# NVIDIA/cuopt

Measured on AMD Instinct MI355X. Metric: pdlp_iterations_per_sec, higher is better.
Workload: dtype f64; 1 GPU; c3: synthetic random sparse LP S(m=1000000,n=1000000,k=10,seed=2), nnz=10000000, longest row 10, CSR fp64/int32, Stable2 preset, tolerances 0 (fixed iteration budget); rows=1000000, cols=1000000, nnz=10000000, parallelism=single GPU

## Files before the change

cuopt_amd/csrc/pdlp_create.hip:

```cpp
#include "pdlp_ctx.hpp"
#include "pdlp_layouts.hpp"
#include "pdlp_setup.hpp"

__global__ void k_fill(int64_t n, double* __restrict__ d, double v);
int sync_panel_values(pdlpdev_ctx* c);
int resident_tier(int m, int n, int64_t nnz);

static thread_local int g_create_sharded = 0;
static thread_local int g_create_no_resident = 0;
static thread_local int g_create_batch_lanes = 0;

static int create_impl(pdlpdev_ctx** out, int device, int32_t m, int32_t n, const int32_t* a_offsets,
                       const int32_t* a_indices, const double* a_values, const int32_t* at_offsets,
                       const int32_t* at_indices, const double* at_values,
                       void (*transpose_ready)(void*), void* user, const double* c, const double* lo,
                       const double* hi, const double* lb, const double* ub, pdlpdev_analysis* an);

extern "C" {

const char* pdlpdev_last_error(void) { return g_err.c_str(); }
void pdlpdev_create_hint(int sharded) { g_create_sharded = sharded; }
void pdlpdev_create_no_resident(int no_resident) { g_create_no_resident = no_resident; }
void pdlpdev_create_batch_lanes(int lanes) { g_create_batch_lanes = lanes; }
static thread_local pdlpdev_ctx* g_create_stream_donor = nullptr;
// ... 446 lines not shown
    lap("wait for the A^T side");
    if ((int64_t)at_offsets[n] != ctx->nnz) return fail(-1, "pdlpdev_create: A and A^T disagree on nnz");
    if (!an) {
      TRY(upload_i32(ctx, &ctx->At.full.off, at_offsets, (size_t)n + 1));
      TRY(upload_i32(ctx, &ctx->At.full.idx, at_indices, nnz, 8));
      TRY(upload_f64(ctx, &ctx->At.full.val, at_values, nnz, 8));
    }
    ctx->At.nlong = (int)lat.size();
    if (ctx->At.nlong) TRY(upload_i32(ctx, &ctx->At.longs, lat.data(), lat.size()));
    const bool hot_t = !hT_off.empty();
    ctx->At.hot = ctx->At.full;
    ctx->At.hot_nnz = (int64_t)T.off[n];
    if (hot_t) {
      TRY(upload_i32(ctx, &ctx->At.hot.off, T.off, (size_t)n + 1));
      TRY(upload_i32(ctx, &ctx->At.hot.idx, T.idx, (size_t)ctx->At.hot_nnz, 8));
      TRY(dev_alloc(ctx, &ctx->At.hot.val, (size_t)ctx->At.hot_nnz + 8));
      TRY(upload_i32(ctx, &ctx->dense.s_perm_at, hT_perm.data(), hT_perm.size()));
    }
    if (DH.on) TRY(dev_alloc(ctx, &ctx->At.dense_add, (size_t)n));
    ctx->At.nb = (int)rbt.size() / 2 - 1;
    TRY(upload_i32(ctx, &ctx->At.rb, rbt.data(), rbt.size()));
    lap("upload A^T");
    T.d_off = ctx->At.hot.off, T.d_idx = ctx->At.hot.idx, T.d_val = ctx->At.hot.val;
    TRY(at_thread ? at_rc : layout_walk(ctx, P, T));
    TRY(upload_side(ctx, P, T));
    if (ctx->At.pan.on && DH.on) TRY(column_segments(ctx, DH, T.ph));
    lap("upload layouts A^T");
    HIP_TRY(hipStreamSynchronize(ctx->stream));
  }
  {
    const char* small_env = getenv("CUOPT_AMD_SMALL");
    const int tier        = resident_tier(m, n, ctx->nnz);
    ctx->eval_reuse_aty   = cuopt_amd::tune_int("eval_reuse_aty", 1) != 0;
    ctx->small_resident   = tier >= 0 && !(small_env && atoi(small_env) == 0) && !ctx->A.dense_add && !ctx->At.dense_add && !g_create_no_resident;
    g_create_no_resident  = 0;
    if (small_env && atoi(small_env) != 0 && tier < 0)
      return fail(-1, "CUOPT_AMD_SMALL=1: the LP does not fit the resident kernel (m, n <= 2048, nnz <= 4096 ...)");
  }
  ctx->slab_cap += slab_rest;
  for (pdlpdev_ctx::MatrixSide* s : {&ctx->A, &ctx->At}) {
    s->pan.v.dense_add = s->jag.v.dense_add = s->pb.v.dense_add = s->dense_add;
    if (s->pan.v.dn_own_seg || s->pan.v.dn_pan_ptr) s->pan.v.dense_add = nullptr;
  }
  TRY(lp_alloc_partials(ctx));
  lap("partial buffers");
  k_fill<<<grid_for(m), kBlock, 0, ctx->stream>>>(m, ctx->dr, 1.0);
  k_fill<<<grid_for(n), kBlock, 0, ctx->stream>>>(n, ctx->dc, 1.0);
  HIP_TRY(hipGetLastError());
  lap("fill D");
  TRY(sync_panel_values(ctx));
  lap("panel values (permute)");
  if (P.mode == LayoutPolicy::kTimed) {
    TRY(pick_layout(ctx, &ctx->A, ctx->tmp_n, ctx->tmp_m));
    lap("layout autotune A");
    TRY(pick_layout(ctx, &ctx->At, ctx->tmp_m, ctx->tmp_n));
    lap("layout autotune");
  }
  if (one_gpu && !ctx->small_resident && ctx->A.layout() == pdlpdev_ctx::MatrixSide::kPanel && !ctx->A.pan.v.seg && cuopt_amd::tune_int("zero_skip", 1) != 0) {
    const size_t words = 2 * (((size_t)n + 127) / 128);
    ctx->zs_mode = cuopt_amd::tune_int("zero_skip", 1) == 2 ? 2 : 1;
    TRY(dev_alloc(ctx, &ctx->zcount, (size_t)grid_for(n)));
    TRY(dev_alloc(ctx, &ctx->xmask, words + 2));
    HIP_TRY(hipMemsetAsync(ctx->xmask, 0, (words + 2) * sizeof(unsigned long long), ctx->stream));
  }
  HIP_TRY(hipStreamSynchronize(ctx->stream));
  scratch_free(ctx);
// ... 34 lines not shown
```

cuopt_amd/csrc/pdlp_ctx.hpp:

```cpp
#pragma once
#include <hip/hip_runtime.h>
#include <hip/hip_ext.h>

#include <tuple>
#include <utility>

#include <dlfcn.h>
#include <unistd.h>
#include <mutex>
#include <math.h>
#include <stdarg.h>
#include <stdio.h>
#include <string.h>

#include <algorithm>
#include <chrono>
#include <map>
#include <memory>
#include <string>
#include <vector>

#include "host_parallel.hpp"
#include "pdlp_kernels.hpp"
#include "pdlp_epilogues.hpp"
// ... 296 lines not shown
    }
    int max_partials() const { return std::max({nb, pb.on ? pb.v.B : 0, pan.on ? pan.v.W : 0, jag.on ? jag.v.nblk + jag.v.nlong : 0, 1}); }
    void info(int32_t out[3]) const
    {
      out[0] = layout();
      switch (layout()) {
        case kPb: out[1] = pb.v.B, out[2] = (int)(100.0 * (pb.pad - 1.0) + 0.5); break;
        case kJag: out[1] = jag.v.nblk, out[2] = (int)(100.0 * jag.saving + 0.5); break;
        case kPanel: out[1] = pan.v.W, out[2] = pan.v.S; break;
        default: out[1] = nb, out[2] = 1;
      }
    }
    bool fuses_dense() const { return pan.on && (pan.v.dn_own_seg != nullptr || pan.v.dn_pan_ptr != nullptr); }
  };
  MatrixSide A, At;
  struct Dense {
    bool on = false;
    int nrows = 0, nseg = 0, ntiles = 0;
    int64_t nent = 0;
    int32_t *row = nullptr, *row_seg = nullptr;
    int32_t *seg_row = nullptr, *seg_c0 = nullptr, *seg_len = nullptr, *seg_ptr = nullptr;
    int32_t *ch_seg = nullptr, *ch_k0 = nullptr, *row_ch = nullptr;
    double* ch_part = nullptr;
    int nchunks = 0;
    int32_t *tile_ptr = nullptr, *tile_seg = nullptr, *tile_id = nullptr;
    int32_t *perm = nullptr, *s_perm_a = nullptr, *s_perm_at = nullptr;
    double* val = nullptr;
    int32_t* tile_slot = nullptr;
  } dense;
  double *c = nullptr, *c_u = nullptr;
  double *dr = nullptr, *dc = nullptr;
  bool scaled = false;
  int eval_reuse_aty = 1;
  int batch_lanes = 0;
  bool small_resident = false;
  rccl::comm_t comm = nullptr;
  softcomm::Comm* soft = nullptr;
  std::string comm_key;
  int rank = 0, world = 1;
  bool rsag = false;
  int slice = 0;
  double* rs_buf = nullptr;
  double* rs_scal = nullptr;
  bool owner = false;
  int ypad = 0;
  double* ygather = nullptr;
  MatrixSide Oc;
  struct Halo {
    bool on = false;
    std::vector<int32_t> recv_off[2], recv_cnt[2], send_off[2], send_cnt[2];
    int64_t bytes = 0, bytes_allgather = 0;
  } halo;
  struct P2P {
    bool on = false;
    char* base = nullptr;
    size_t bytes = 0;
    size_t off_x = 0, off_y = 0, off_s = 0, off_f = 0;
    p2pdev::Peers peers{};
    std::vector<void*> opened;
    unsigned long long* epoch = nullptr;
    int* fault = nullptr;
    p2pdev::Push* push_dev = nullptr;
    p2pdev::Push push_host[p2pdev::kKinds];
  } p2p;
};

struct HalpernBurstStats { int64_t bursts = 0, periods = 0, records = 0, empty = 0; };

struct CtxLp {
  double *lb = nullptr, *ub = nullptr, *lo = nullptr, *hi = nullptr;
  double *lb_u = nullptr, *ub_u = nullptr, *lo_u = nullptr, *hi_u = nullptr;
  double *x[2] = {nullptr, nullptr}, *y[2] = {nullptr, nullptr}, *aty[2] = {nullptr, nullptr};
  double *xbar = nullptr, *sumx = nullptr, *sumy = nullptr, *avgx = nullptr, *avgy = nullptr;
  unsigned long long* xmask = nullptr;
  int* zcount = nullptr;
  int zs_mode = 0;
  double *lrx = nullptr, *lry = nullptr, *rc[2] = {nullptr, nullptr};
  double *tmp_n = nullptr, *tmp_m = nullptr;
  double *ax_u[3] = {nullptr, nullptr, nullptr}, *aty_u[3] = {nullptr, nullptr, nullptr};
  double* rc_scratch = nullptr;
  double *bestx = nullptr, *besty = nullptr, *bestrc = nullptr;
  double *part_g = nullptr;
  double *scal = nullptr;
  double *scal_h = nullptr;
  pdlpdev_ctl *ctl = nullptr, *ctl_h = nullptr;
  pdlpdev_step_params sp = {0.3, 0.6, 0.5, 0.5};
  bool halpern = false;
  double* lraty = nullptr;
  pdlpdev_halpern *hal = nullptr, *hal_h = nullptr;
  bool halpern_rays = false;
  struct pdlpdev_halpern_major_state* hmaj = nullptr;
  pdlpdev_halpern_major_record* hmaj_ring = nullptr;
  HalpernBurstStats burst_stats;
  double* ar_buf = nullptr;
  bool prof_armed = false;
  static constexpr int kProfPairs = 8;
  hipEvent_t prof_ev[2 * kProfPairs] = {};
  int prof_used = 0;
  int rejected_in_a_row = 0;
  bool aty_valid = false, ctl_h_current = false;
  bool batch_ctl_fresh = false;
  int batch_ray_steps = -1, batch_ray_rule = -1;
  int64_t stat_single_rays = 0;
  int spare_attempts = 0;
  int64_t stat_eval_reused = 0, stat_eval_product = 0, stat_loop_syncs = 0, stat_empty_attempts = 0;
  int64_t stat_scaling[2][9] = {};
  int use_graph = 1;
  bool comm_warm = false;
  bool graph_comm_failed = false;
// ... 261 lines not shown
```

cuopt_amd/csrc/pdlp_device.hip:

```cpp
#include "pdlp_ctx.hpp"
#include "pdlp_layouts.hpp"
#include "pdlp_setup.hpp"
#include "halpern_decision.hpp"


__global__ void __launch_bounds__(kBlock) k_fill(int64_t n, double* __restrict__ d, double v)
{
  for (int64_t i = blockIdx.x * (int64_t)kBlock + threadIdx.x; i < n; i += (int64_t)gridDim.x * kBlock)
    d[i] = v;
}
__global__ void __launch_bounds__(kBlock) k_scale_vectors(int n, int m, double* __restrict__ c,
                                                          double* __restrict__ lb,
                                                          double* __restrict__ ub,
                                                          const double* __restrict__ dc,
                                                          double* __restrict__ lo,
                                                          double* __restrict__ hi,
                                                          const double* __restrict__ dr)
{
  const int tot = n > m ? n : m;
  for (int i = blockIdx.x * kBlock + threadIdx.x; i < tot; i += gridDim.x * kBlock) {
    if (i < n) {
      c[i]  = c[i] * dc[i];
      lb[i] = lb[i] / dc[i];
      ub[i] = ub[i] / dc[i];
// ... 52 lines not shown
    } else if (MODE == 1) {
      acc[0] += a[i] * a[i];
    } else if (MODE == 2) {
      const double v = combine_bounds(a[i], b[i]);
      acc[0] += v * v;
    } else {
      const double v = a[i] - b[i];
      acc[0] += v * v;
    }
  }
  if (MODE == 0)
    block_reduce<MaxOp, 1>(acc, red);
  else
    block_reduce<SumOp, 1>(acc, red);
  if (threadIdx.x == 0) part[blockIdx.x] = acc[0];
}
__global__ void __launch_bounds__(kBlock) k_dot(int64_t n, const double* __restrict__ a, const double* __restrict__ b,
                                                double* __restrict__ part)
{
  __shared__ double red[8];
  double acc[1] = {0.0};
  for (int64_t i = blockIdx.x * (int64_t)kBlock + threadIdx.x; i < n; i += (int64_t)gridDim.x * kBlock) acc[0] += a[i] * b[i];
  block_reduce<SumOp, 1>(acc, red);
  if (threadIdx.x == 0) part[blockIdx.x] = acc[0];
}
__global__ void __launch_bounds__(kBlock) k_finalize(const double* __restrict__ part, int nb, int nq,
                                                     unsigned op_mask, double* __restrict__ out)
{
  __shared__ double red[8];
  finalize_rows(part, nb, nq, op_mask, out, red);
}

template <bool ZS>
__device__ __forceinline__ void
primal_body(int n, const pdlpdev_ctl* __restrict__ ctl, double* __restrict__ x0, double* __restrict__ x1,
         const double* __restrict__ aty0, const double* __restrict__ aty1,
         const double* __restrict__ c, const double* __restrict__ lb, const double* __restrict__ ub,
         double* __restrict__ xbar, double* __restrict__ sumx, const p2pdev::Push* __restrict__ push, pdlpdev_ctx::UniformBounds ubd,
         unsigned long long* __restrict__ xmask, int* __restrict__ zcount)
{
  [[maybe_unused]] int nz = 0;
  if (!loop_active(ctl)) return;
  const int cur       = ctl->cur;
  const double tau    = ctl->tau;
  const double weight = ctl->step_size;
  const bool pend     = ctl->pending_avg != 0;
  const double* __restrict__ x   = cur ? x1 : x0;
  double* __restrict__ xn        = cur ? x0 : x1;
  const double* __restrict__ aty = cur ? aty1 : aty0;
  for (int j = blockIdx.x * kBlock + threadIdx.x; j < n; j += gridDim.x * kBlock) {
    const double xj       = x[j];
    const double gradient = c[j] - aty[j];
    double next           = xj - (tau * gradient);
    next                  = dmax(dmin(next, ubd.ub_same ? ubd.ub : ub[j]), ubd.lb_same ? ubd.lb : lb[j]);
    xn[j]                 = next;
    const double xb       = next - xj + next;
    xbar[j]               = xb;
    if constexpr (ZS) {
      const unsigned long long bits = __ballot(xb != 0.0);
      if ((threadIdx.x & 63) == 0) xmask[j >> 6] = bits;
      nz += __popcll(bits);
    }
    if (push)
      for (int q = 0; q < push->world; ++q)
        if (push->wants(q, j)) p2pdev::put(push->slot(q) + j, xb);
    if (pend) sumx[j] = sumx[j] + weight * xj;
  }
  if constexpr (ZS) {
    __shared__ int wave_nz[kBlock / 64];
    if ((threadIdx.x & 63) == 0) wave_nz[threadIdx.x >> 6] = nz;
    __syncthreads();
    if (threadIdx.x == 0) {
      int sum = 0;
#pragma unroll
      for (int w = 0; w < kBlock / 64; ++w) sum += wave_nz[w];
      zcount[blockIdx.x] = sum;
    }
  }
  if (push) p2pdev::count_exchange(push);
}
__global__ void __launch_bounds__(kBlock)
k_primal(int n, const pdlpdev_ctl* __restrict__ ctl, double* __restrict__ x0, double* __restrict__ x1,
         const double* __restrict__ aty0, const double* __restrict__ aty1,
         const double* __restrict__ c, const double* __restrict__ lb, const double* __restrict__ ub,
         double* __restrict__ xbar, double* __restrict__ sumx, const p2pdev::Push* __restrict__ push, pdlpdev_ctx::UniformBounds ubd)
{
  primal_body<false>(n, ctl, x0, x1, aty0, aty1, c, lb, ub, xbar, sumx, push, ubd, nullptr, nullptr);
}
__global__ void __launch_bounds__(kBlock)
k_primal_zs(int n, const pdlpdev_ctl* __restrict__ ctl, double* __restrict__ x0, double* __restrict__ x1,
            const double* __restrict__ aty0, const double* __restrict__ aty1,
            const double* __restrict__ c, const double* __restrict__ lb, const double* __restrict__ ub,
            double* __restrict__ xbar, double* __restrict__ sumx, pdlpdev_ctx::UniformBounds ubd,
            unsigned long long* __restrict__ xmask, int* __restrict__ zcount)
{
  primal_body<true>(n, ctl, x0, x1, aty0, aty1, c, lb, ub, xbar, sumx, nullptr, ubd, xmask, zcount);
}



__global__ void __launch_bounds__(kBlock)
k_step_stats(int n, int nbg, const pdlpdev_ctl* __restrict__ ctl, const double* __restrict__ reduced,
             const double* __restrict__ x0, const double* __restrict__ x1, double* __restrict__ aty0,
             double* __restrict__ aty1, double* __restrict__ part)
{
  __shared__ double red[12];
  if (!loop_active(ctl)) return;
  const int cur = ctl->cur;
  const double* __restrict__ x   = cur ? x1 : x0;
  const double* __restrict__ xn  = cur ? x0 : x1;
  const double* __restrict__ aty = cur ? aty1 : aty0;
  double* __restrict__ atyn      = cur ? aty0 : aty1;
  double acc[2] = {0.0, 0.0};
  for (int j = blockIdx.x * kBlock + threadIdx.x; j < n; j += gridDim.x * kBlock) {
    const double v  = reduced[j];
    atyn[j]         = v;
    const double dx = xn[j] - x[j];
    const double t  = v - aty[j];
    acc[0] += t * dx;
    acc[1] += dx * dx;
  }
  block_reduce<SumOp, 2>(acc, red);
  if (threadIdx.x == 0) {
    part[blockIdx.x]       = acc[0];
    part[nbg + blockIdx.x] = acc[1];
  }
}

constexpr int kDecisionThreads = 1024;
static_assert(kDecisionThreads == kHalpernDecisionThreads, "k_halpern_decision runs halpern_decision_workgroup");
template <bool ZS = false>
__device__ __forceinline__ void step_decision_workgroup(pdlpdev_ctl* __restrict__ ctl, const double* __restrict__ part_dy, int nb_dy,
                                                        const double* __restrict__ part_t, int nb_t, const double* __restrict__ dy2_reduced,
                                                        const pdlpdev_step_params& sp, const int* __restrict__ zcount = nullptr, int nb_z = 0,
                                                        int zn = 0, int zmode = 0)
{
  __shared__ double red[(ZS ? 4 : 3) * 16];
  __shared__ double pw[2];
  pdlpdev_ctl lc = *ctl;
  if (!(lc.error == 0 && lc.steps_taken < lc.target_steps)) return;
  const int t = threadIdx.x;
  if (t >= kDecisionThreads - 2) {
    const double knext = (double)(lc.k + 1) + 1.0;
    pw[t - (kDecisionThreads - 2)] = pow(knext, t == kDecisionThreads - 2 ? -sp.reduction_exponent : -sp.growth_exponent);
  }
  double acc[ZS ? 4 : 3] = {0.0, 0.0, 0.0};
  if (dy2_reduced == nullptr) {
#pragma unroll 4
    for (int i = t; i < nb_dy; i += kDecisionThreads) acc[0] += part_dy[i];
  }
#pragma unroll 4
  for (int i = t; i < nb_t; i += kDecisionThreads) {
    acc[1] += part_t[i];
    acc[2] += part_t[nb_t + i];
  }
  if constexpr (ZS) {
    acc[3] = 0.0;
#pragma unroll 2
    for (int i = t; i < nb_z; i += kDecisionThreads) acc[3] += (double)zcount[i];
  }
  block_sum_fast<ZS ? 4 : 3, kDecisionThreads / 64>(acc, red);
  if (t != 0) return;
  apply_step_decision(&lc, dy2_reduced ? dy2_reduced[0] : acc[0], acc[1], acc[2], sp, pw);
  if constexpr (ZS) {
    const long long nonzeros = (long long)acc[3];
    lc.zs_nonzeros           = (int32_t)nonzeros;
    if (zmode == 2 || nonzeros * 4 <= 3ll * zn) lc.zskip = 1;
    else if (nonzeros * 100 >= 87ll * zn) lc.zskip = 0;
    *ctl = lc;
  } else {
    __builtin_memcpy(ctl, &lc, offsetof(pdlpdev_ctl, zskip));
  }
}
__global__ void __launch_bounds__(kDecisionThreads)
k_step_decision(pdlpdev_ctl* __restrict__ ctl, const double* __restrict__ part_dy, int nb_dy,
                const double* __restrict__ part_t, int nb_t, const double* __restrict__ dy2_reduced,
                pdlpdev_step_params sp)
{
  step_decision_workgroup(ctl, part_dy, nb_dy, part_t, nb_t, dy2_reduced, sp);
}
__global__ void __launch_bounds__(kDecisionThreads)
k_step_decision_zs(pdlpdev_ctl* __restrict__ ctl, const double* __restrict__ part_dy, int nb_dy,
                   const double* __restrict__ part_t, int nb_t, pdlpdev_step_params sp, const int* __restrict__ zcount, int nb_z, int zn, int zmode)
{
  step_decision_workgroup<true>(ctl, part_dy, nb_dy, part_t, nb_t, nullptr, sp, zcount, nb_z, zn, zmode);
}
__global__ void __launch_bounds__(kDecisionThreads)
k_step_decision_batch(const pdlpdev_decision_args* __restrict__ args)
{
  const pdlpdev_decision_args a = args[blockIdx.x];
  step_decision_workgroup(a.ctl, a.part_dy, a.nb_dy, a.part_t, a.nb_t, nullptr, a.sp);
}

__global__ void __launch_bounds__(kDecisionThreads)
k_halpern_decision(pdlpdev_ctl* __restrict__ ctl, pdlpdev_halpern* __restrict__ hal, const double* __restrict__ part_dy, int nb_dy,
                   const double* __restrict__ part_t, int nb_t)
{
  halpern_decision_workgroup(ctl, hal, part_dy, nb_dy, part_t, nb_t);
}
__global__ void k_halpern_clear(pdlpdev_halpern* hal)
{
  hal->r = hal->r_first = hal->r2 = 0.0;
  hal->r2_min = __builtin_huge_val();
  hal->k = 0, hal->reserved = 0;
}
__global__ void k_halpern_restart_ctl(pdlpdev_ctl* ctl, pdlpdev_halpern* hal, double* dist2, double theta)
{
  halpern_restart_scalars(ctl, hal, dist2, theta);
}
__global__ void __launch_bounds__(kBlock)
k_copy_current(int n, const pdlpdev_ctl* __restrict__ ctl, const double* __restrict__ v0, const double* __restrict__ v1, double* __restrict__ out)
{
  const double* __restrict__ v = ctl->cur ? v1 : v0;
  for (int i = blockIdx.x * kBlock + threadIdx.x; i < n; i += gridDim.x * kBlock) out[i] = v[i];
}
__global__ void __launch_bounds__(kBlock) k_div_by_scalar(int n, double* __restrict__ out, const double* __restrict__ v, double d)
{
  for (int i = blockIdx.x * kBlock + threadIdx.x; i < n; i += gridDim.x * kBlock) out[i] = v[i] / d;
}

__device__ __forceinline__ bool p2p_exchange_step_sums(pdlpdev_ctl* __restrict__ ctl, const double* __restrict__ part_dy, int nb_dy,
                                                       const double* __restrict__ part_t, int nb_t, const double* __restrict__ landed,
                                                       const unsigned long long* __restrict__ flags, int world,
                                                       const unsigned long long* __restrict__ epoch, int* __restrict__ fault,
// ... 623 lines not shown
    return launch_k(ctx, k_primal_zs, grid_for(n), kBlock, 0, n, ctx->ctl, ctx->x[0], ctx->x[1], ctx->aty[0], ctx->aty[1], ctx->c, ctx->lb, ctx->ub, ctx->xbar, ctx->sumx, ctx->ubd, xmask, ctx->zcount);
  launch_primal_slice(ctx, ColSlice{0, n}, nullptr);
}
static void launch_a_dual(pdlpdev_ctx* ctx, double* ycopy = nullptr, const p2pdev::Push* push = nullptr)
{
  ctx->A.pan.v.zmask = attempt_xmask(ctx), ctx->A.pan.v.zcols = ctx->n, ctx->A.pan.v.zforce = ctx->zs_mode == 2;
  const Gathered g = Gathered::fixed(ctx->xbar, true);
  const auto pre  = std::make_tuple(ctx->ctl);
  const auto vecs = std::make_tuple(ctx->xbar);
  if (ctx->halpern && ycopy)
    (void)launch_product(ctx, ctx->A, products::a_halpern_sharded, g, pre, vecs, std::make_tuple(ctx->y[0], ctx->y[1], ctx->lo, ctx->hi, halpern_args(ctx), ctx->A.part, ycopy, push));
  else if (ctx->halpern) (void)launch_product(ctx, ctx->A, products::a_halpern, g, pre, vecs, std::make_tuple(ctx->y[0], ctx->y[1], ctx->lo, ctx->hi, halpern_args(ctx), ctx->A.part));
  else (void)launch_product(ctx, ctx->A, products::a_dual, g, pre, vecs, std::make_tuple(ctx->y[0], ctx->y[1], ctx->lo, ctx->hi, ctx->sumy, ctx->A.part, ycopy, push));
}
static void launch_at_step(pdlpdev_ctx* ctx)
{
  const auto pre = std::make_tuple(ctx->ctl);
  if (ctx->halpern)
    (void)launch_product(ctx, ctx->At, products::at_halpern, Gathered::fixed(ctx->avgy, true), pre, std::make_tuple(),
                         std::make_tuple(ctx->x[0], ctx->x[1], ctx->aty[0], ctx->aty[1], halpern_args(ctx), ctx->At.part));
  else
    (void)launch_product(ctx, ctx->At, products::at_step, Gathered::trial(ctx->y[0], ctx->y[1], true), pre, std::make_tuple(ctx->y[0], ctx->y[1]),
                         std::make_tuple(ctx->x[0], ctx->x[1], ctx->aty[0], ctx->aty[1], ctx->At.part));
}
void launch_at_cur(pdlpdev_ctx* ctx, double* out_override, int use_next)
{
  (void)launch_product(ctx, ctx->At, products::at_cur, use_next ? Gathered::trial(ctx->y[0], ctx->y[1]) : Gathered::current(ctx->y[0], ctx->y[1]), std::make_tuple(ctx->ctl),
                       std::make_tuple(ctx->y[0], ctx->y[1]), std::make_tuple(ctx->aty[0], ctx->aty[1], out_override, use_next));
}
void launch_plain(pdlpdev_ctx* ctx, int transpose, const double* vec, double* out)
{
  (void)launch_product(ctx, transpose ? ctx->At : ctx->A, products::plain, Gathered::fixed(vec), std::make_tuple(), std::make_tuple(vec), std::make_tuple(out));
}
static void launch_decision(pdlpdev_ctx* ctx)
{
  if (ctx->halpern) return launch_k(ctx, k_halpern_decision, 1, kDecisionThreads, 0, ctx->ctl, ctx->hal, ctx->A.part, ctx->A.partials(), ctx->At.part, ctx->At.partials());
  if (attempt_xmask(ctx))
    return launch_k(ctx, k_step_decision_zs, 1, kDecisionThreads, 0, ctx->ctl, ctx->A.part, ctx->A.partials(), ctx->At.part, ctx->At.partials(), ctx->sp, ctx->zcount,
                    grid_for(ctx->n), ctx->n, ctx->zs_mode);
  launch_k(ctx, k_step_decision, 1, kDecisionThreads, 0, ctx->ctl, ctx->A.part, ctx->A.partials(), ctx->At.part, ctx->At.partials(), nullptr, ctx->sp);
}

static void launch_oc_step(pdlpdev_ctx* ctx, const ColSlice& sl)
{
  const size_t cs = sl.cs;
  double *x0 = ctx->x[0] + cs, *x1 = ctx->x[1] + cs, *t0 = ctx->aty[0] + cs, *t1 = ctx->aty[1] + cs;
  const double* yg = ctx->ygather;
  if (ctx->halpern) {
    const HalpernArgs h{ctx->hal, ctx->ar_buf + cs , const_cast<double*>(yg), ctx->lrx + cs, ctx->lry, ctx->lraty + cs};
    (void)launch_product(ctx, ctx->Oc, products::at_halpern, Gathered::fixed(yg, true), std::make_tuple(ctx->ctl), std::make_tuple(),
                         std::make_tuple(x0, x1, t0, t1, h, ctx->Oc.part));
    return;
  }
  (void)launch_product(ctx, ctx->Oc, products::at_step, Gathered::trial(yg, yg, true), std::make_tuple(ctx->ctl), std::make_tuple(yg, yg),
                       std::make_tuple(x0, x1, t0, t1, ctx->Oc.part));
}

static void launch_decision_reduced(pdlpdev_ctx* ctx, const double* part_t, int nb_t, const double* dy2)
{
  launch_k(ctx, k_step_decision, 1, kDecisionThreads, 0, ctx->ctl, nullptr, 0, part_t, nb_t, dy2, ctx->sp);
}

struct AttemptStage { int id; void (*launch)(pdlpdev_ctx*); };
static const AttemptStage kSingleStages[4] = {{PDLPDEV_K_PRIMAL, launch_primal}, {PDLPDEV_K_SPMV_A_DUAL, [](pdlpdev_ctx* c) { launch_a_dual(c); }},
                                              {PDLPDEV_K_SPMV_AT_STEP, launch_at_step}, {PDLPDEV_K_STEP_DECISION, launch_decision}};
static int enqueue_single(pdlpdev_ctx* ctx)
{
  for (const AttemptStage& st : kSingleStages) st.launch(ctx);
  LAUNCH_CHECK();
  return 0;
}
static int enqueue_replicated(pdlpdev_ctx* ctx)
{
  const int n = ctx->n, g = std::min(grid_for(n), kGenericBlocks);
  launch_primal(ctx);
  launch_a_dual(ctx);
  launch_at_cur(ctx, ctx->ar_buf, 1);
  launch_k(ctx, k_sum_partials_to, 1, kBlock, 0, ctx->A.part, ctx->A.partials(), ctx->ar_buf + n);
  LAUNCH_CHECK();
  TRY(allreduce(ctx, ctx->ar_buf, (size_t)n + 1, rccl::kSum));
  launch_k(ctx, k_step_stats, g, kBlock, 0, n, g, ctx->ctl, ctx->ar_buf, ctx->x[0], ctx->x[1], ctx->aty[0], ctx->aty[1], ctx->part_g);
  launch_decision_reduced(ctx, ctx->part_g, g, ctx->ar_buf + n);
  LAUNCH_CHECK();
  return 0;
}
static int enqueue_rsag(pdlpdev_ctx* ctx)
{
  const ColSlice sl = rank_slice(ctx);
  const int g       = std::min(grid_for(sl.len), kGenericBlocks);
  launch_primal_slice(ctx, sl, nullptr);
  LAUNCH_CHECK();
  TRY(all_gather(ctx, ctx->xbar, (size_t)ctx->slice));
  launch_a_dual(ctx);
  launch_at_cur(ctx, ctx->ar_buf, 1);
  LAUNCH_CHECK();
  TRY(reduce_scatter(ctx, ctx->ar_buf, ctx->rs_buf, (size_t)ctx->slice));
  launch_k(ctx, k_step_stats, g, kBlock, 0, sl.len, g, ctx->ctl, ctx->rs_buf, ctx->x[0] + sl.cs, ctx->x[1] + sl.cs, ctx->aty[0] + sl.cs, ctx->aty[1] + sl.cs, ctx->part_g);
  launch_k(ctx, k_pack_step_sums, 1, kBlock, 0, ctx->A.part, ctx->A.partials(), ctx->part_g, g, ctx->rs_scal);
  LAUNCH_CHECK();
  TRY(allreduce(ctx, ctx->rs_scal, 3, rccl::kSum));
  launch_decision_reduced(ctx, ctx->rs_scal + 1, 1, ctx->rs_scal);
// ... 31 lines not shown
                    P.fault, P.push_dev + kind);
  }
  const int count = ctx->world * per_rank, remote = count - per_rank;
  const int g     = std::max(1, std::min((remote + 4095) / 4096, 1024));
  launch_k(ctx, p2pdev::k_pull, g, 256, 0, ctx->ctl, dst, land, count, ctx->rank * per_rank, per_rank, p2p_flags(P), ctx->world, kind, P.epoch, P.fault, P.push_dev + kind);
}
static int enqueue_owner_p2p(pdlpdev_ctx* ctx)
{
  pdlpdev_ctx::P2P& P = ctx->p2p;
  const ColSlice sl   = rank_slice(ctx);
  const double* sums  = reinterpret_cast<const double*>(P.base + P.off_s);
  launch_primal_slice(ctx, sl, P.push_dev);
  LAUNCH_CHECK();
  p2p_pull(ctx, 0, ctx->xbar, P.off_x, ctx->slice);
  launch_a_dual(ctx, ctx->ygather + (size_t)ctx->rank * ctx->ypad, P.push_dev + 1);
  p2p_pull(ctx, 1, ctx->ygather, P.off_y, ctx->ypad);
  launch_oc_step(ctx, sl);
  if (ctx->halpern) launch_k(ctx, k_halpern_decision_p2p, 1, kBlock, 0, ctx->ctl, ctx->hal, ctx->A.part, ctx->A.partials(), ctx->Oc.part, ctx->Oc.partials(), sums, p2p_flags(P),
                             ctx->world, P.epoch, P.fault, P.push_dev + 2);
  else launch_k(ctx, k_step_decision_p2p, 1, kBlock, 0, ctx->ctl, ctx->A.part, ctx->A.partials(), ctx->Oc.part, ctx->Oc.partials(), sums, p2p_flags(P), ctx->world, P.epoch,
                P.fault, ctx->sp, P.push_dev + 2);
  LAUNCH_CHECK();
  return 0;
}

static int enqueue_attempt(pdlpdev_ctx* ctx)
{
  if (ctx->halpern && ctx->comm && !ctx->owner) return fail(-7, "reflected Halpern mode: behind a communicator the owner-computes dataflow only");
  if (ctx->owner && !ctx->Oc.hot.off) return fail(-1, "owner-computes dataflow: pdlpdev_owner_setup was not called");
  if (ctx->owner) return ctx->p2p.on ? enqueue_owner_p2p(ctx) : enqueue_owner_collective(ctx);
  if (ctx->rsag) return enqueue_rsag(ctx);
  return ctx->comm ? enqueue_replicated(ctx) : enqueue_single(ctx);
}

static int get_graph(pdlpdev_ctx* ctx, int attempts, hipGraphExec_t* out)
{
  auto it = ctx->graphs.find(attempts);
  if (it != ctx->graphs.end()) {
    *out = it->second;
    return 0;
  }
  hipGraph_t graph;
  HIP_TRY(hipStreamBeginCapture(ctx->stream, hipStreamCaptureModeThreadLocal));
  int rc = 0;
  for (int i = 0; i < attempts && rc == 0; ++i) rc = enqueue_attempt(ctx);
  hipError_t e = hipStreamEndCapture(ctx->stream, &graph);
  if (rc != 0) return rc;
  HIP_TRY(e);
  hipGraphExec_t exec;
  HIP_TRY(hipGraphInstantiate(&exec, graph, nullptr, nullptr, 0));
  HIP_TRY(hipGraphDestroy(graph));
  ctx->graphs[attempts] = exec;
  *out                  = exec;
  return 0;
}

static int enqueue_attempts(pdlpdev_ctx* ctx, int remaining)
{
  const bool rccl_graphs = ctx->comm && !ctx->p2p.on && !ctx->soft && !ctx->graph_comm_failed;
  bool replayed = false;
  if (rccl_graphs && ctx->use_graph && !ctx->comm_warm) {
    TRY(enqueue_attempt(ctx));
    ctx->comm_warm = true;
    remaining -= 1;
  }
  if (ctx->use_graph && (!ctx->comm || ctx->p2p.on || rccl_graphs)) {
    replayed = true;
    while (remaining > 0) {
      const int chunk = attempt_chunk(remaining);
      hipGraphExec_t g;
      const int grc = get_graph(ctx, chunk, &g);
      if (grc != 0 && rccl_graphs) {
        ctx->graph_comm_failed = true;
        (void)hipGetLastError();
        replayed = false;
        break;
      }
      TRY(grc);
      HIP_TRY(hipGraphLaunch(g, ctx->stream));
      remaining -= chunk;
    }
  }
  if (!replayed) {
    for (int i = 0; i < remaining; ++i) TRY(enqueue_attempt(ctx));
  }
  return 0;
}

static void note_attempts(pdlpdev_ctx* ctx, int before, int attempts_before, int enqueued)
{
  const pdlpdev_ctl& c = *ctx->ctl_h;
  const int made       = c.attempts - attempts_before;
  if (!ctx->comm) ctx->stat_empty_attempts += enqueued - made;
  if (c.steps_taken > before && c.error == 0 && !ctx->comm) ctx->aty_valid = true;
  if (c.error != 0) ctx->aty_valid = false;
}
static int after_round(pdlpdev_ctx* ctx, int before, int attempts_before, int enqueued, int counted )
{
  note_attempts(ctx, before, attempts_before, enqueued);
  if (ctx->p2p.on && ctx->ctl_h->error != 0) {
    int fault = 0;
    HIP_TRY(hipMemcpy(&fault, ctx->p2p.fault, sizeof(int), hipMemcpyDeviceToHost));
    if (fault) return fail(-6, "direct peer transport: rank %d waited 5 s for another rank's data (a peer failed or is stuck)", ctx->rank);
  }
  if (too_many_rejections(ctx, before, counted)) {
    k_set_error<<<1, 1, 0, ctx->stream>>>(ctx->ctl);
    LAUNCH_CHECK();
    TRY(fetch_ctl_counted(ctx, nullptr));
    ctx->aty_valid = false;
  }
  return 0;
}
static int run_round(pdlpdev_ctx* ctx, int attempts_before, int enqueue, int counted)
{
  const int before = ctx->ctl_h->steps_taken;
  TRY(enqueue_attempts(ctx, enqueue));
  TRY(fetch_ctl_counted(ctx, nullptr));
// ... 703 lines not shown
```

Before: 6902 iterations/s.

## Fuse step decision into next primal update kernel within captured attempt chunks

```diff
diff --git a/cuopt_amd/csrc/pdlp_create.hip b/cuopt_amd/csrc/pdlp_create.hip
--- a/cuopt_amd/csrc/pdlp_create.hip
+++ b/cuopt_amd/csrc/pdlp_create.hip
@@ -502,6 +502,9 @@
     const char* small_env = getenv("CUOPT_AMD_SMALL");
     const int tier        = resident_tier(m, n, ctx->nnz);
     ctx->eval_reuse_aty   = cuopt_amd::tune_int("eval_reuse_aty", 1) != 0;
+    const long long decides_key = cuopt_amd::tune_int("primal_decides", -1);
+    ctx->primal_decides   = decides_key < 0 ? n >= pdlpdev_ctx::kPrimalDecidesMinCols : decides_key != 0;
+    ctx->primal_decide_grid_cap = (int)std::max<long long>(1, std::min<long long>(cuopt_amd::tune_int("primal_decide_grid", 512), 512));
     ctx->small_resident   = tier >= 0 && !(small_env && atoi(small_env) == 0) && !ctx->A.dense_add && !ctx->At.dense_add && !g_create_no_resident;
     g_create_no_resident  = 0;
     if (small_env && atoi(small_env) != 0 && tier < 0)
diff --git a/cuopt_amd/csrc/pdlp_ctx.hpp b/cuopt_amd/csrc/pdlp_ctx.hpp
--- a/cuopt_amd/csrc/pdlp_ctx.hpp
+++ b/cuopt_amd/csrc/pdlp_ctx.hpp
@@ -352,6 +352,9 @@
   double *dr = nullptr, *dc = nullptr;
   bool scaled = false;
   int eval_reuse_aty = 1;
+  static constexpr int kPrimalDecidesMinCols = 786432;
+  int primal_decides = 1;
+  int primal_decide_grid_cap = 512;
   int batch_lanes = 0;
   bool small_resident = false;
   rccl::comm_t comm = nullptr;
@@ -395,6 +398,8 @@
   unsigned long long* xmask = nullptr;
   int* zcount = nullptr;
   int zs_mode = 0;
+  pdlpdev_ctl* chunk_ctl[2] = {nullptr, nullptr};
+  int* zcount_alt = nullptr;
   double *lrx = nullptr, *lry = nullptr, *rc[2] = {nullptr, nullptr};
   double *tmp_n = nullptr, *tmp_m = nullptr;
   double *ax_u[3] = {nullptr, nullptr, nullptr}, *aty_u[3] = {nullptr, nullptr, nullptr};
diff --git a/cuopt_amd/csrc/pdlp_device.hip b/cuopt_amd/csrc/pdlp_device.hip
--- a/cuopt_amd/csrc/pdlp_device.hip
+++ b/cuopt_amd/csrc/pdlp_device.hip
@@ -108,6 +108,36 @@
 }
 
 template <bool ZS>
+__device__ __forceinline__ double primal_column(int j, double xj, double cj, double atyj, double lbj, double ubj, double tau, double* __restrict__ xn,
+                                                double* __restrict__ xbar, unsigned long long* __restrict__ xmask, int& nz)
+{
+  const double gradient = cj - atyj;
+  double next           = xj - (tau * gradient);
+  next                  = dmax(dmin(next, ubj), lbj);
+  xn[j]                 = next;
+  const double xb       = next - xj + next;
+  xbar[j]               = xb;
+  if constexpr (ZS) {
+    const unsigned long long bits = __ballot(xb != 0.0);
+    if ((threadIdx.x & 63) == 0) xmask[j >> 6] = bits;
+    nz += __popcll(bits);
+  }
+  return xb;
+}
+template <int WAVES>
+__device__ __forceinline__ void primal_store_zcount(int nz, int* __restrict__ zcount)
+{
+  __shared__ int wave_nz[WAVES];
+  if ((threadIdx.x & 63) == 0) wave_nz[threadIdx.x >> 6] = nz;
+  __syncthreads();
+  if (threadIdx.x == 0) {
+    int sum = 0;
+#pragma unroll
+    for (int w = 0; w < WAVES; ++w) sum += wave_nz[w];
+    zcount[blockIdx.x] = sum;
+  }
+}
+template <bool ZS>
 __device__ __forceinline__ void
 primal_body(int n, const pdlpdev_ctl* __restrict__ ctl, double* __restrict__ x0, double* __restrict__ x1,
          const double* __restrict__ aty0, const double* __restrict__ aty1,
@@ -125,34 +155,14 @@
   double* __restrict__ xn        = cur ? x0 : x1;
   const double* __restrict__ aty = cur ? aty1 : aty0;
   for (int j = blockIdx.x * kBlock + threadIdx.x; j < n; j += gridDim.x * kBlock) {
-    const double xj       = x[j];
-    const double gradient = c[j] - aty[j];
-    double next           = xj - (tau * gradient);
-    next                  = dmax(dmin(next, ubd.ub_same ? ubd.ub : ub[j]), ubd.lb_same ? ubd.lb : lb[j]);
-    xn[j]                 = next;
-    const double xb       = next - xj + next;
-    xbar[j]               = xb;
-    if constexpr (ZS) {
-      const unsigned long long bits = __ballot(xb != 0.0);
-      if ((threadIdx.x & 63) == 0) xmask[j >> 6] = bits;
-      nz += __popcll(bits);
-    }
+    const double xj = x[j];
+    const double xb = primal_column<ZS>(j, xj, c[j], aty[j], ubd.lb_same ? ubd.lb : lb[j], ubd.ub_same ? ubd.ub : ub[j], tau, xn, xbar, xmask, nz);
     if (push)
       for (int q = 0; q < push->world; ++q)
         if (push->wants(q, j)) p2pdev::put(push->slot(q) + j, xb);
     if (pend) sumx[j] = sumx[j] + weight * xj;
   }
-  if constexpr (ZS) {
-    __shared__ int wave_nz[kBlock / 64];
-    if ((threadIdx.x & 63) == 0) wave_nz[threadIdx.x >> 6] = nz;
-    __syncthreads();
-    if (threadIdx.x == 0) {
-      int sum = 0;
-#pragma unroll
-      for (int w = 0; w < kBlock / 64; ++w) sum += wave_nz[w];
-      zcount[blockIdx.x] = sum;
-    }
-  }
+  if constexpr (ZS) primal_store_zcount<kBlock / 64>(nz, zcount);
   if (push) p2pdev::count_exchange(push);
 }
 __global__ void __launch_bounds__(kBlock)
@@ -205,67 +215,193 @@
 
 constexpr int kDecisionThreads = 1024;
 static_assert(kDecisionThreads == kHalpernDecisionThreads, "k_halpern_decision runs halpern_decision_workgroup");
-template <bool ZS = false>
-__device__ __forceinline__ void step_decision_workgroup(pdlpdev_ctl* __restrict__ ctl, const double* __restrict__ part_dy, int nb_dy,
-                                                        const double* __restrict__ part_t, int nb_t, const double* __restrict__ dy2_reduced,
-                                                        const pdlpdev_step_params& sp, const int* __restrict__ zcount = nullptr, int nb_z = 0,
-                                                        int zn = 0, int zmode = 0)
+template <bool ZS, bool EVERY, class Ahead>
+__device__ __forceinline__ void step_decision_form(pdlpdev_ctl& lc, const double* __restrict__ part_dy, int nb_dy, const double* __restrict__ part_t, int nb_t,
+                                                   const double* __restrict__ dy2_reduced, const pdlpdev_step_params& sp, const int* __restrict__ zcount,
+                                                   int nb_z, int zn, int zmode, Ahead&& ahead)
 {
   __shared__ double red[(ZS ? 4 : 3) * 16];
   __shared__ double pw[2];
-  pdlpdev_ctl lc = *ctl;
-  if (!(lc.error == 0 && lc.steps_taken < lc.target_steps)) return;
   const int t = threadIdx.x;
+  const bool has_dy = dy2_reduced == nullptr && t < nb_dy, has_t = t < nb_t, has_z = ZS && t < nb_z;
+  const int i_t = min(t, nb_t - 1);
+  const double first_dy = dy2_reduced == nullptr && nb_dy > 0 ? part_dy[min(t, nb_dy - 1)] : 0.0;
+  const double first_t0 = nb_t > 0 ? part_t[i_t] : 0.0, first_t1 = nb_t > 0 ? part_t[nb_t + i_t] : 0.0;
+  [[maybe_unused]] int first_z = 0;
+  if constexpr (ZS) first_z = nb_z > 0 ? zcount[min(t, nb_z - 1)] : 0;
+  ahead();
   if (t >= kDecisionThreads - 2) {
     const double knext = (double)(lc.k + 1) + 1.0;
     pw[t - (kDecisionThreads - 2)] = pow(knext, t == kDecisionThreads - 2 ? -sp.reduction_exponent : -sp.growth_exponent);
   }
-  double acc[ZS ? 4 : 3] = {0.0, 0.0, 0.0};
+  double zero = 0.0;
+  int izero   = 0;
+  asm volatile("" : "+v"(zero), "+v"(izero));
+  double acc[ZS ? 4 : 3] = {zero, zero, zero};
   if (dy2_reduced == nullptr) {
+    if (has_dy) acc[0] += first_dy;
 #pragma unroll 4
-    for (int i = t; i < nb_dy; i += kDecisionThreads) acc[0] += part_dy[i];
-  }
+    for (int i = t + kDecisionThreads; i < nb_dy; i += kDecisionThreads) acc[0] += part_dy[i];
+  }
+  if (has_t) acc[1] += first_t0, acc[2] += first_t1;
 #pragma unroll 4
-  for (int i = t; i < nb_t; i += kDecisionThreads) {
+  for (int i = t + kDecisionThreads; i < nb_t; i += kDecisionThreads) {
     acc[1] += part_t[i];
     acc[2] += part_t[nb_t + i];
   }
   if constexpr (ZS) {
-    acc[3] = 0.0;
+    acc[3] = zero;
+    if (has_z) acc[3] += (double)(first_z + izero);
 #pragma unroll 2
-    for (int i = t; i < nb_z; i += kDecisionThreads) acc[3] += (double)zcount[i];
+    for (int i = t + kDecisionThreads; i < nb_z; i += kDecisionThreads) acc[3] += (double)zcount[i];
   }
   block_sum_fast<ZS ? 4 : 3, kDecisionThreads / 64>(acc, red);
-  if (t != 0) return;
+  if (!EVERY && t != 0) return;
   apply_step_decision(&lc, dy2_reduced ? dy2_reduced[0] : acc[0], acc[1], acc[2], sp, pw);
   if constexpr (ZS) {
     const long long nonzeros = (long long)acc[3];
     lc.zs_nonzeros           = (int32_t)nonzeros;
     if (zmode == 2 || nonzeros * 4 <= 3ll * zn) lc.zskip = 1;
     else if (nonzeros * 100 >= 87ll * zn) lc.zskip = 0;
-    *ctl = lc;
+  }
+}
+template <bool ZS>
+__device__ __forceinline__ void store_ctl(pdlpdev_ctl* out, const pdlpdev_ctl& lc)
+{
+  if constexpr (ZS) {
+    *out = lc;
   } else {
-    __builtin_memcpy(ctl, &lc, offsetof(pdlpdev_ctl, zskip));
-  }
+    __builtin_memcpy(out, &lc, offsetof(pdlpdev_ctl, zskip));
+  }
+}
+template <bool ZS = false>
+__device__ __forceinline__ void step_decision_workgroup(const pdlpdev_ctl* in, pdlpdev_ctl* out, const double* __restrict__ part_dy, int nb_dy,
+                                                        const double* __restrict__ part_t, int nb_t, const double* __restrict__ dy2_reduced,
+                                                        const pdlpdev_step_params& sp, const int* __restrict__ zcount = nullptr, int nb_z = 0,
+                                                        int zn = 0, int zmode = 0)
+{
+  pdlpdev_ctl lc = *in;
+  if (!(lc.error == 0 && lc.steps_taken < lc.target_steps)) {
+    if (in != out && threadIdx.x == 0) store_ctl<ZS>(out, lc);
+    return;
+  }
+  step_decision_form<ZS, false>(lc, part_dy, nb_dy, part_t, nb_t, dy2_reduced, sp, zcount, nb_z, zn, zmode, [] {});
+  if (threadIdx.x == 0) store_ctl<ZS>(out, lc);
 }
 __global__ void __launch_bounds__(kDecisionThreads)
-k_step_decision(pdlpdev_ctl* __restrict__ ctl, const double* __restrict__ part_dy, int nb_dy,
+k_step_decision(const pdlpdev_ctl* in, pdlpdev_ctl* out, const double* __restrict__ part_dy, int nb_dy,
                 const double* __restrict__ part_t, int nb_t, const double* __restrict__ dy2_reduced,
                 pdlpdev_step_params sp)
 {
-  step_decision_workgroup(ctl, part_dy, nb_dy, part_t, nb_t, dy2_reduced, sp);
+  step_decision_workgroup(in, out, part_dy, nb_dy, part_t, nb_t, dy2_reduced, sp);
 }
 __global__ void __launch_bounds__(kDecisionThreads)
-k_step_decision_zs(pdlpdev_ctl* __restrict__ ctl, const double* __restrict__ part_dy, int nb_dy,
+k_step_decision_zs(const pdlpdev_ctl* in, pdlpdev_ctl* out, const double* __restrict__ part_dy, int nb_dy,
                    const double* __restrict__ part_t, int nb_t, pdlpdev_step_params sp, const int* __restrict__ zcount, int nb_z, int zn, int zmode)
 {
-  step_decision_workgroup<true>(ctl, part_dy, nb_dy, part_t, nb_t, nullptr, sp, zcount, nb_z, zn, zmode);
+  step_decision_workgroup<true>(in, out, part_dy, nb_dy, part_t, nb_t, nullptr, sp, zcount, nb_z, zn, zmode);
+}
+
+constexpr int kPrimalDecideCols = 4;
+constexpr int kPrimalDecideMaxGrid = 512;
+static inline int primal_decide_grid(int n, int cap)
+{
+  const int per = kDecisionThreads * kPrimalDecideCols;
+  return std::max(1, std::min((n + per - 1) / per, cap));
+}
+template <bool ZS>
+__device__ __forceinline__ void
+primal_decide_body(int n, const pdlpdev_ctl* in, pdlpdev_ctl* out, double* __restrict__ x0, double* __restrict__ x1,
+                   const double* __restrict__ aty0, const double* __restrict__ aty1, const double* __restrict__ c, const double* __restrict__ lb,
+                   const double* __restrict__ ub, double* __restrict__ xbar, double* __restrict__ sumx, pdlpdev_ctx::UniformBounds ubd,
+                   unsigned long long* __restrict__ xmask, int* __restrict__ zcount_out, const double* __restrict__ part_dy, int nb_dy,
+                   const double* __restrict__ part_t, int nb_t, const pdlpdev_step_params& sp, const int* __restrict__ zcount_in, int nb_z, int zmode)
+{
+  constexpr int U = kPrimalDecideCols, T = kDecisionThreads;
+  [[maybe_unused]] int nz = 0;
+  pdlpdev_ctl lc = *in;
+  if (!(lc.error == 0 && lc.steps_taken < lc.target_steps)) {
+    if (blockIdx.x == 0 && threadIdx.x == 0) store_ctl<ZS>(out, lc);
+    return;
+  }
+  const int ahead = lc.cur ^ 1;
+  const int j0    = blockIdx.x * (U * T) + threadIdx.x;
+  double xj[U], tj[U], cj[U], sj[U], lbj[U], ubj[U];
+  step_decision_form<ZS, true>(lc, part_dy, nb_dy, part_t, nb_t, nullptr, sp, zcount_in, nb_z, n, zmode, [&] {
+#pragma unroll
+    for (int u = 0; u < U; ++u) {
+      const int j = min(j0 + u * T, n - 1);
+      xj[u]  = (ahead ? x1 : x0)[j];
+      tj[u]  = (ahead ? aty1 : aty0)[j];
+      cj[u]  = c[j];
+      sj[u]  = sumx[j];
+    }
+#pragma unroll
+    for (int u = 0; u < U; ++u) lbj[u] = ubd.lb_same ? ubd.lb : lb[min(j0 + u * T, n - 1)];
+#pragma unroll
+    for (int u = 0; u < U; ++u) ubj[u] = ubd.ub_same ? ubd.ub : ub[min(j0 + u * T, n - 1)];
+  });
+  if (blockIdx.x == 0 && threadIdx.x == 0) store_ctl<ZS>(out, lc);
+  if (!(lc.error == 0 && lc.steps_taken < lc.target_steps)) return;
+  const int cur       = __builtin_amdgcn_readfirstlane(lc.cur);
+  const bool pend     = __builtin_amdgcn_readfirstlane(lc.pending_avg) != 0;
+  const double tau    = lc.tau;
+  const double weight = lc.step_size;
+  const double* __restrict__ x   = cur ? x1 : x0;
+  double* __restrict__ xn        = cur ? x0 : x1;
+  const double* __restrict__ aty = cur ? aty1 : aty0;
+  if (cur != ahead) {
+#pragma unroll
+    for (int u = 0; u < U; ++u) {
+      const int j = j0 + u * T;
+      if (j < n) xj[u] = x[j], tj[u] = aty[j];
+    }
+  }
+#pragma unroll
+  for (int u = 0; u < U; ++u) {
+    const int j = j0 + u * T;
+    if (j < n) {
+      primal_column<ZS>(j, xj[u], cj[u], tj[u], lbj[u], ubj[u], tau, xn, xbar, xmask, nz);
+      if (pend) sumx[j] = sj[u] + weight * xj[u];
+    }
+  }
+  for (long long base = ((long long)blockIdx.x + gridDim.x) * (U * T); base < n; base += (long long)gridDim.x * (U * T)) {
+#pragma unroll
+    for (int u = 0; u < U; ++u) {
+      const long long jj = base + threadIdx.x + u * T;
+      if (jj < n) {
+        const int j = (int)jj;
+        const double xv = x[j];
+        primal_column<ZS>(j, xv, c[j], aty[j], ubd.lb_same ? ubd.lb : lb[j], ubd.ub_same ? ubd.ub : ub[j], tau, xn, xbar, xmask, nz);
+        if (pend) sumx[j] = sumx[j] + weight * xv;
+      }
+    }
+  }
+  if constexpr (ZS) primal_store_zcount<T / 64>(nz, zcount_out);
+}
+__global__ void __launch_bounds__(kDecisionThreads)
+k_primal_decide(int n, const pdlpdev_ctl* in, pdlpdev_ctl* out, double* __restrict__ x0, double* __restrict__ x1,
+                const double* __restrict__ aty0, const double* __restrict__ aty1, const double* __restrict__ c, const double* __restrict__ lb,
+                const double* __restrict__ ub, double* __restrict__ xbar, double* __restrict__ sumx, pdlpdev_ctx::UniformBounds ubd,
+                const double* __restrict__ part_dy, int nb_dy, const double* __restrict__ part_t, int nb_t, pdlpdev_step_params sp)
+{
+  primal_decide_body<false>(n, in, out, x0, x1, aty0, aty1, c, lb, ub, xbar, sumx, ubd, nullptr, nullptr, part_dy, nb_dy, part_t, nb_t, sp, nullptr, 0, 0);
+}
+__global__ void __launch_bounds__(kDecisionThreads)
+k_primal_decide_zs(int n, const pdlpdev_ctl* in, pdlpdev_ctl* out, double* __restrict__ x0, double* __restrict__ x1,
+                   const double* __restrict__ aty0, const double* __restrict__ aty1, const double* __restrict__ c, const double* __restrict__ lb,
+                   const double* __restrict__ ub, double* __restrict__ xbar, double* __restrict__ sumx, pdlpdev_ctx::UniformBounds ubd,
+                   unsigned long long* __restrict__ xmask, int* __restrict__ zcount_out, const double* __restrict__ part_dy, int nb_dy,
+                   const double* __restrict__ part_t, int nb_t, pdlpdev_step_params sp, const int* __restrict__ zcount_in, int nb_z, int zmode)
+{
+  primal_decide_body<true>(n, in, out, x0, x1, aty0, aty1, c, lb, ub, xbar, sumx, ubd, xmask, zcount_out, part_dy, nb_dy, part_t, nb_t, sp, zcount_in, nb_z,
+                           zmode);
 }
 __global__ void __launch_bounds__(kDecisionThreads)
 k_step_decision_batch(const pdlpdev_decision_args* __restrict__ args)
 {
   const pdlpdev_decision_args a = args[blockIdx.x];
-  step_decision_workgroup(a.ctl, a.part_dy, a.nb_dy, a.part_t, a.nb_t, nullptr, a.sp);
+  step_decision_workgroup(a.ctl, a.ctl, a.part_dy, a.nb_dy, a.part_t, a.nb_t, nullptr, a.sp);
 }
 
 __global__ void __launch_bounds__(kDecisionThreads)
@@ -955,13 +1091,26 @@
 {
   (void)launch_product(ctx, transpose ? ctx->At : ctx->A, products::plain, Gathered::fixed(vec), std::make_tuple(), std::make_tuple(vec), std::make_tuple(out));
 }
+static void launch_decision_into(pdlpdev_ctx* ctx, pdlpdev_ctl* out, const int* zc, int nb_z)
+{
+  if (attempt_xmask(ctx))
+    return launch_k(ctx, k_step_decision_zs, 1, kDecisionThreads, 0, ctx->ctl, out, ctx->A.part, ctx->A.partials(), ctx->At.part, ctx->At.partials(), ctx->sp, zc, nb_z,
+                    ctx->n, ctx->zs_mode);
+  launch_k(ctx, k_step_decision, 1, kDecisionThreads, 0, ctx->ctl, out, ctx->A.part, ctx->A.partials(), ctx->At.part, ctx->At.partials(), nullptr, ctx->sp);
+}
 static void launch_decision(pdlpdev_ctx* ctx)
 {
   if (ctx->halpern) return launch_k(ctx, k_halpern_decision, 1, kDecisionThreads, 0, ctx->ctl, ctx->hal, ctx->A.part, ctx->A.partials(), ctx->At.part, ctx->At.partials());
-  if (attempt_xmask(ctx))
-    return launch_k(ctx, k_step_decision_zs, 1, kDecisionThreads, 0, ctx->ctl, ctx->A.part, ctx->A.partials(), ctx->At.part, ctx->At.partials(), ctx->sp, ctx->zcount,
-                    grid_for(ctx->n), ctx->n, ctx->zs_mode);
-  launch_k(ctx, k_step_decision, 1, kDecisionThreads, 0, ctx->ctl, ctx->A.part, ctx->A.partials(), ctx->At.part, ctx->At.partials(), nullptr, ctx->sp);
+  launch_decision_into(ctx, ctx->ctl, ctx->zcount, grid_for(ctx->n));
+}
+static void launch_primal_decide(pdlpdev_ctx* ctx, const pdlpdev_ctl* in, pdlpdev_ctl* out, const int* zc_in, int nb_z, int* zc_out)
+{
+  const int n = ctx->n;
+  if (unsigned long long* xmask = attempt_xmask(ctx))
+    return launch_k(ctx, k_primal_decide_zs, primal_decide_grid(n, ctx->primal_decide_grid_cap), kDecisionThreads, 0, n, in, out, ctx->x[0], ctx->x[1], ctx->aty[0], ctx->aty[1], ctx->c, ctx->lb, ctx->ub,
+                    ctx->xbar, ctx->sumx, ctx->ubd, xmask, zc_out, ctx->A.part, ctx->A.partials(), ctx->At.part, ctx->At.partials(), ctx->sp, zc_in, nb_z, ctx->zs_mode);
+  launch_k(ctx, k_primal_decide, primal_decide_grid(n, ctx->primal_decide_grid_cap), kDecisionThreads, 0, n, in, out, ctx->x[0], ctx->x[1], ctx->aty[0], ctx->aty[1], ctx->c, ctx->lb, ctx->ub, ctx->xbar,
+           ctx->sumx, ctx->ubd, ctx->A.part, ctx->A.partials(), ctx->At.part, ctx->At.partials(), ctx->sp);
 }
 
 static void launch_oc_step(pdlpdev_ctx* ctx, const ColSlice& sl)
@@ -981,7 +1130,7 @@
 
 static void launch_decision_reduced(pdlpdev_ctx* ctx, const double* part_t, int nb_t, const double* dy2)
 {
-  launch_k(ctx, k_step_decision, 1, kDecisionThreads, 0, ctx->ctl, nullptr, 0, part_t, nb_t, dy2, ctx->sp);
+  launch_k(ctx, k_step_decision, 1, kDecisionThreads, 0, ctx->ctl, ctx->ctl, nullptr, 0, part_t, nb_t, dy2, ctx->sp);
 }
 
 struct AttemptStage { int id; void (*launch)(pdlpdev_ctx*); };
@@ -990,6 +1139,47 @@
 static int enqueue_single(pdlpdev_ctx* ctx)
 {
   for (const AttemptStage& st : kSingleStages) st.launch(ctx);
+  LAUNCH_CHECK();
+  return 0;
+}
+static bool chunk_decides_in_primal(const pdlpdev_ctx* ctx) { return ctx->primal_decides && !ctx->halpern && !ctx->comm && !ctx->small_resident && ctx->n > 0; }
+static int chunk_blocks_ready(pdlpdev_ctx* ctx)
+{
+  if (!chunk_decides_in_primal(ctx) || ctx->chunk_ctl[0]) return 0;
+  TRY(dev_alloc(ctx, &ctx->chunk_ctl[0], 1));
+  TRY(dev_alloc(ctx, &ctx->chunk_ctl[1], 1));
+  if (ctx->zcount) {
+    TRY(dev_alloc(ctx, &ctx->zcount_alt, (size_t)grid_for(ctx->n)));
+  }
+  return 0;
+}
+static int enqueue_single_chunk(pdlpdev_ctx* ctx, int attempts)
+{
+  if (!chunk_decides_in_primal(ctx) || attempts == 1) {
+    for (int k = 0; k < attempts; ++k) TRY(enqueue_single(ctx));
+    return 0;
+  }
+  if (!ctx->chunk_ctl[0]) return fail(-1, "enqueue_single_chunk: chunk_blocks_ready was not called");
+  struct ChunkBlocks {
+    pdlpdev_ctx* c;
+    pdlpdev_ctl* const home;
+    ~ChunkBlocks() { c->ctl = home; }
+  } blocks{ctx, ctx->ctl};
+  int* const zc[2] = {ctx->zcount, ctx->zcount_alt};
+  int nb_z         = grid_for(ctx->n);
+  for (int k = 0; k < attempts; ++k) {
+    if (k == 0) {
+      launch_primal(ctx);
+    } else {
+      pdlpdev_ctl* const decided = ctx->chunk_ctl[k & 1];
+      launch_primal_decide(ctx, ctx->ctl, decided, zc[(k - 1) & 1], nb_z, zc[k & 1]);
+      ctx->ctl = decided;
+      nb_z     = primal_decide_grid(ctx->n, ctx->primal_decide_grid_cap);
+    }
+    launch_a_dual(ctx);
+    launch_at_step(ctx);
+  }
+  launch_decision_into(ctx, blocks.home, zc[(attempts - 1) & 1], nb_z);
   LAUNCH_CHECK();
   return 0;
 }
@@ -1087,6 +1277,12 @@
   if (ctx->rsag) return enqueue_rsag(ctx);
   return ctx->comm ? enqueue_replicated(ctx) : enqueue_single(ctx);
 }
+static int enqueue_chunk(pdlpdev_ctx* ctx, int attempts)
+{
+  if (!ctx->comm && !ctx->owner && !ctx->rsag) return enqueue_single_chunk(ctx, attempts);
+  for (int i = 0; i < attempts; ++i) TRY(enqueue_attempt(ctx));
+  return 0;
+}
 
 static int get_graph(pdlpdev_ctx* ctx, int attempts, hipGraphExec_t* out)
 {
@@ -1095,10 +1291,10 @@
     *out = it->second;
     return 0;
   }
+  TRY(chunk_blocks_ready(ctx));
   hipGraph_t graph;
   HIP_TRY(hipStreamBeginCapture(ctx->stream, hipStreamCaptureModeThreadLocal));
-  int rc = 0;
-  for (int i = 0; i < attempts && rc == 0; ++i) rc = enqueue_attempt(ctx);
+  const int rc = enqueue_chunk(ctx, attempts);
   hipError_t e = hipStreamEndCapture(ctx->stream, &graph);
   if (rc != 0) return rc;
   HIP_TRY(e);
@@ -1136,8 +1332,9 @@
       remaining -= chunk;
     }
   }
-  if (!replayed) {
-    for (int i = 0; i < remaining; ++i) TRY(enqueue_attempt(ctx));
+  if (!replayed && remaining > 0) {
+    TRY(chunk_blocks_ready(ctx));
+    TRY(enqueue_chunk(ctx, remaining));
   }
   return 0;
 }
```

Measured after the change: 7016 iterations/s, median of 6. 1.6% higher.
